# mpeg5/xevd

Hardware: AMD Instinct MI355X
Metric: frames/sec (bit-exact YUV) + achieved HBM GB/s (higher is better)
Workload: dtype s16; 1 GPU; cfg4_main_8k_10b_ra; width=7680, height=4320, bit_depth=10, batches_resident=4, residual_pass_ahead=True, parallelism=1 stream on 1 GPU

## Files before the change

xevd_amd/csrc/itdq_body.h:

```cpp
#pragma once
#include "xgpu_internal.h"

typedef short v2s __attribute__((ext_vector_type(2)));

static __constant__ uint32_t k_tmp[2730];
__host__ __device__ constexpr int tmp_base(int log2n) { return log2n == 1 ? 0 : log2n == 2 ? 2 : log2n == 3 ? 10 : log2n == 4 ? 42 : log2n == 5 ? 170 : 682; }

static __constant__ uint32_t k_atsp[2][680];
__host__ __device__ constexpr int atsp_base(int log2n) { return log2n == 2 ? 0 : log2n == 3 ? 8 : log2n == 4 ? 40 : 168; }

static void upload_transform_tables_tu(const int *tm, const int16_t *ats, hipStream_t s)
{
    static uint32_t apk[2][680];
    for (int t = 0; t < 2; t++) {
        int src = 0;
        for (int l = 2; l <= 5; l++) {
            const int N = 1 << l, dst = atsp_base(l);
            for (int k2 = 0; k2 < N / 2; k2++)
                for (int n = 0; n < N; n++)
                    apk[t][dst + k2 * N + n] = (uint32_t)(uint16_t)ats[t * 1360 + src + (2 * k2) * N + n] |
                                               ((uint32_t)(uint16_t)ats[t * 1360 + src + (2 * k2 + 1) * N + n] << 16);
            src += N * N;
        }
    }
    (void)hipMemcpyToSymbolAsync(HIP_SYMBOL(k_atsp), apk, sizeof(apk), 0, hipMemcpyHostToDevice, s);
    static uint32_t packed[2730];
    int src = 0;
    for (int l = 1; l <= 6; l++) {
        const int N = 1 << l, dst = tmp_base(l);
        for (int k2 = 0; k2 < N / 2; k2++)
            for (int n = 0; n < N; n++)
                packed[dst + k2 * N + n] = (uint32_t)(uint16_t)(int16_t)tm[src + (2 * k2) * N + n] |
                                           ((uint32_t)(uint16_t)(int16_t)tm[src + (2 * k2 + 1) * N + n] << 16);
        src += N * N;
    }
    (void)hipMemcpyToSymbolAsync(HIP_SYMBOL(k_tmp), packed, sizeof(packed), 0, hipMemcpyHostToDevice, s);
    (void)hipStreamSynchronize(s);
}

__device__ __forceinline__ int clip16(int v) { return min(max(v, -32768), 32767); }
__device__ __forceinline__ int dot2(uint32_t a, uint32_t b, int c)
{
    return __builtin_amdgcn_sdot2(__builtin_bit_cast(v2s, a), __builtin_bit_cast(v2s, b), c, false);
}

__host__ __device__ constexpr int itdq_group(int lw, int lh)
{
    const int W = 1 << lw, H = 1 << lh;
    const int l1 = W * (H > 16 ? H / 16 : 1), l2 = H * (W > 16 ? W / 16 : 1);
    return 256 / (l1 > l2 ? l1 : l2);
}

#define ITDQ_PLANES_DWORDS 4608
#define ITDQ_LDS_DWORDS (ITDQ_PLANES_DWORDS + 2048)
#define ITDQ_MAX_G 128

__device__ __forceinline__ uint32_t wave_or(uint32_t v)
{
#pragma unroll
    for (int m = 32; m >= 1; m >>= 1) v |= (uint32_t)__shfl_xor((int)v, m, 64);
    return v;
}

template <int LW, int LH, bool IQT>
__device__ __forceinline__ void itdq_item(const ItdqArgs &a, const TbWave wv, uint32_t *lds, uint32_t *s_rm, uint32_t *s_cm)
{
    constexpr int W = 1 << LW, H = 1 << LH;
    constexpr int N1 = H > 16 ? 16 : H, C1 = H / N1;
    constexpr int N2 = W > 16 ? 16 : W, C2 = W / N2;
    constexpr int G = itdq_group(LW, LH);
    constexpr int RS = W / 2 + 1;
    constexpr int PLANE = G * H * RS;
    constexpr bool UNI1 = (G * W) % 64 == 0, UNI2 = (G * H) % 64 == 0;
    static_assert(2 * PLANE <= ITDQ_PLANES_DWORDS && G * W * H <= 4096 && G <= ITDQ_MAX_G, "LDS budget");
    constexpr int PLANES_DWORDS = IQT ? ITDQ_PLANES_DWORDS / 2 : ITDQ_PLANES_DWORDS;
    constexpr bool RMASK = H >= 16, CMASK = W >= 16;
    const int t = threadIdx.x;
    if (RMASK || CMASK) {
        if (t < G) { s_rm[t] = 0; s_cm[t] = 0; }
        __syncthreads();
    }
    const uint32_t *tmh = (wv.tr_v == TR_DCT2 || LH < 2 || LH > 5) ? k_tmp + tmp_base(LH) : k_atsp[wv.tr_v - 1] + atsp_base(LH);
    const uint32_t *tmw = (wv.tr_h == TR_DCT2 || LW < 2 || LW > 5) ? k_tmp + tmp_base(LW) : k_atsp[wv.tr_h - 1] + atsp_base(LW);
    const bool s16_mid = IQT || wv.tr_v != TR_DCT2 || wv.tr_h != TR_DCT2;
    int16_t *ldsh = (int16_t *)lds;
    int16_t *ldsl = (int16_t *)(lds + PLANE);
    uint32_t *ldsc = lds + PLANES_DWORDS;

    {
        constexpr int S = W * H, UN = S >= 8 ? 8 : 4;
        constexpr int odd = (LW + LH) & 1;
        const int shift = 20 - 14 - (15 - a.bd - ((LW + LH) >> 1)) + (odd ? 8 : 0);
        const long long offset = shift == 0 ? 0 : 1ll << (shift - 1);
        for (int u = t; u < G * S / UN; u += 256) {
            const int p = (u * UN) / S, o = (u * UN) % S;
            if (p >= wv.count) break;
            const TbRec tb = a.tbs[wv.first + p];
            const int qp = tb.qp, sidx = qp % 6;
            const int sbase = sidx == 0 ? 40 : sidx == 1 ? 45 : sidx == 2 ? 51 : sidx == 3 ? 57 : sidx == 4 ? 64 : (IQT ? 72 : 71);
            const long long mul = (long long)(sbase << (qp / 6)) * (odd ? 181 : 1);
            const int16_t *src = a.coef + tb.off + ((o >> LW) << tb.log2s) + (o & (W - 1));
            uint32_t raw[UN / 2];
            if constexpr (UN == 8) { const uint4 v = *(const uint4 *)src; raw[0] = v.x; raw[1] = v.y; raw[2] = v.z; raw[3] = v.w; }
            else { const uint2 v = *(const uint2 *)src; raw[0] = v.x; raw[1] = v.y; }
#pragma unroll
            for (int i = 0; i < UN / 2; i++) {
                if (raw[i] == 0) continue;
                const int c0 = (int16_t)(raw[i] & 0xFFFF), c1 = (int16_t)(raw[i] >> 16);
                const long long l0 = ((long long)c0 * mul + offset) >> shift, l1 = ((long long)c1 * mul + offset) >> shift;
                const int v0 = (int)min(max(l0, -32768ll), 32767ll), v1 = (int)min(max(l1, -32768ll), 32767ll);
                raw[i] = (uint32_t)(uint16_t)v0 | ((uint32_t)(uint16_t)v1 << 16);
                if (RMASK) atomicOr(&s_rm[p], 1u << ((o + 2 * i) >> (LW + 1)));
                if (CMASK) atomicOr(&s_cm[p], 1u << (((o + 2 * i) & (W - 1)) >> 1));
            }
#pragma unroll
            for (int i = 0; i < UN / 2; i++) ldsc[(p * S + o) / 2 + i] = raw[i];
        }
    }
    __syncthreads();

    uint32_t rows1 = 0;
    if (RMASK) {
        const int p1 = (t % (G * W)) >> LW;
        rows1 = (uint32_t)__builtin_amdgcn_readfirstlane((int)wave_or((t < G * W * C1 && p1 < wv.count) ? s_rm[p1] : 0u));
    }
    if (t < G * W * C1) {
        const int idx = t % (G * W);
        int chunk = t / (G * W);
        if (UNI1) chunk = __builtin_amdgcn_readfirstlane(chunk);
        const int p = idx >> LW, j = idx & (W - 1);
        const bool valid = p < wv.count;
        const int16_t *src = (const int16_t *)ldsc + p * (W * H) + j;

        int acc[N1];
#pragma unroll
        for (int n = 0; n < N1; n++) acc[n] = 0;
        if (RMASK) {
            for (uint32_t m = rows1; m; m &= m - 1) {
                const int k2 = __builtin_ctz(m);
                const uint32_t vp = valid ? ((uint32_t)(uint16_t)src[(2 * k2) * W] | ((uint32_t)(uint16_t)src[(2 * k2 + 1) * W] << 16)) : 0u;
                const uint32_t *row = tmh + k2 * H + chunk * N1;
#pragma unroll
                for (int n = 0; n < N1; n++) acc[n] = dot2(row[n], vp, acc[n]);
            }
        } else {
            for (int k2 = 0; k2 < H / 2; k2++) {
                const uint32_t vp = valid ? ((uint32_t)(uint16_t)src[(2 * k2) * W] | ((uint32_t)(uint16_t)src[(2 * k2 + 1) * W] << 16)) : 0u;
                if (__ballot(vp != 0) == 0) continue;
                const uint32_t *row = tmh + k2 * H + chunk * N1;
#pragma unroll
                for (int n = 0; n < N1; n++) acc[n] = dot2(row[n], vp, acc[n]);
            }
        }
        const int base = (p * H + chunk * N1) * (2 * RS) + j;
        if (CMASK && !(valid && ((s_cm[p] >> (j >> 1)) & 1))) {
        } else if (s16_mid) {
#pragma unroll
            for (int n = 0; n < N1; n++) ldsh[base + n * (2 * RS)] = (int16_t)clip16((acc[n] + 64) >> 7);
        } else {
#pragma unroll
            for (int n = 0; n < N1; n++) {
                ldsh[base + n * (2 * RS)] = (int16_t)(acc[n] >> 15);
                ldsl[base + n * (2 * RS)] = (int16_t)(acc[n] & 0x7FFF);
            }
        }
    }
    __syncthreads();

    uint32_t cols2 = 0;
    if (CMASK) {
        const int p2 = (t % (G * H)) >> LH;
        cols2 = (uint32_t)__builtin_amdgcn_readfirstlane((int)wave_or((t < G * H * C2 && p2 < wv.count) ? s_cm[p2] : 0u));
    }
    if (t < G * H * C2) {
        const int idx = t % (G * H);
        int chunk = t / (G * H);
        if (UNI2) chunk = __builtin_amdgcn_readfirstlane(chunk);
        const int p = idx >> LH, r = idx & (H - 1);
        if (p >= wv.count) return;
        const uint32_t own = CMASK ? s_cm[p] : 0xFFFFFFFFu;
        const TbRec tb = a.tbs[wv.first + p];
        const int shift2 = s16_mid ? 12 - (a.bd - 8) : 7 + 12 - (a.bd - 8);
        const uint32_t *inh = lds + (p * H + r) * RS;
        const uint32_t *inl = inh + PLANE;
        int res[N2];
        if (s16_mid) {
            int s[N2];
#pragma unroll
            for (int n = 0; n < N2; n++) s[n] = 1 << (shift2 - 1);
            if (CMASK) {
                for (uint32_t m = cols2; m; m &= m - 1) {
                    const int k2 = __builtin_ctz(m);
                    const uint32_t vp = ((own >> k2) & 1) ? inh[k2] : 0u;
                    const uint32_t *row = tmw + k2 * W + chunk * N2;
#pragma unroll
                    for (int n = 0; n < N2; n++) s[n] = dot2(row[n], vp, s[n]);
                }
            } else {
                for (int k2 = 0; k2 < W / 2; k2++) {
                    const uint32_t vp = inh[k2];
                    if (__ballot(vp != 0) == 0) continue;
                    const uint32_t *row = tmw + k2 * W + chunk * N2;
#pragma unroll
                    for (int n = 0; n < N2; n++) s[n] = dot2(row[n], vp, s[n]);
                }
            }
#pragma unroll
            for (int n = 0; n < N2; n++) res[n] = clip16(s[n] >> shift2);
        } else {
            int sh[N2], sl[N2];
#pragma unroll
            for (int n = 0; n < N2; n++) { sh[n] = 0; sl[n] = 0; }
            if (CMASK) {
                for (uint32_t m = cols2; m; m &= m - 1) {
                    const int k2 = __builtin_ctz(m);
                    const bool mine = (own >> k2) & 1;
                    const uint32_t vh = mine ? inh[k2] : 0u, vl = mine ? inl[k2] : 0u;
                    const uint32_t *row = tmw + k2 * W + chunk * N2;
#pragma unroll
                    for (int n = 0; n < N2; n++) { sh[n] = dot2(row[n], vh, sh[n]); sl[n] = dot2(row[n], vl, sl[n]); }
                }
            } else {
                for (int k2 = 0; k2 < W / 2; k2++) {
                    const uint32_t vh = inh[k2], vl = inl[k2];
                    if (__ballot((vh | vl) != 0) == 0) continue;
                    const uint32_t *row = tmw + k2 * W + chunk * N2;
#pragma unroll
                    for (int n = 0; n < N2; n++) { sh[n] = dot2(row[n], vh, sh[n]); sl[n] = dot2(row[n], vl, sl[n]); }
                }
            }
            const long long add = 1ll << (shift2 - 1);
#pragma unroll
            for (int n = 0; n < N2; n++) {
                const long long s = (long long)sh[n] * 32768 + sl[n] + add;
                res[n] = (int)min(max(s >> shift2, -32768ll), 32767ll);
            }
        }
        int16_t *out = a.resid + tb.off + (r << tb.log2s) + chunk * N2;
        if constexpr (N2 >= 8) {
#pragma unroll
            for (int n = 0; n < N2; n += 8) {
                uint4 v;
                v.x = (uint32_t)(uint16_t)res[n + 0] | ((uint32_t)(uint16_t)res[n + 1] << 16);
                v.y = (uint32_t)(uint16_t)res[n + 2] | ((uint32_t)(uint16_t)res[n + 3] << 16);
                v.z = (uint32_t)(uint16_t)res[n + 4] | ((uint32_t)(uint16_t)res[n + 5] << 16);
                v.w = (uint32_t)(uint16_t)res[n + 6] | ((uint32_t)(uint16_t)res[n + 7] << 16);
                *(uint4 *)(out + n) = v;
            }
        } else if constexpr (N2 == 4) {
            uint2 v;
            v.x = (uint32_t)(uint16_t)res[0] | ((uint32_t)(uint16_t)res[1] << 16);
            v.y = (uint32_t)(uint16_t)res[2] | ((uint32_t)(uint16_t)res[3] << 16);
            *(uint2 *)out = v;
        } else {
            *(uint32_t *)out = (uint32_t)(uint16_t)res[0] | ((uint32_t)(uint16_t)res[1] << 16);
        }
    }
}

template <bool IQT>
__device__ __forceinline__ void itdq_dispatch(const ItdqArgs &a, int wi, uint32_t *lds, uint32_t *s_rm, uint32_t *s_cm)
{
    const TbWave wv = a.waves[wi];
#define CASE(lw, lh) case (lw) * 8 + (lh): itdq_item<lw, lh, IQT>(a, wv, lds, s_rm, s_cm); break;
#define ROW(lw) CASE(lw, 1) CASE(lw, 2) CASE(lw, 3) CASE(lw, 4) CASE(lw, 5) CASE(lw, 6)
    switch (wv.log2w * 8 + wv.log2h) {
        ROW(1) ROW(2) ROW(3) ROW(4) ROW(5) ROW(6)
        default: break;
    }
#undef ROW
#undef CASE
}
```

xevd_amd/csrc/k_intra.hip:

```cpp
#include "xgpu_internal.h"
#include "itdq_body.h"

#include <type_traits>
#include "intra_pred.h"

#define INTRA_WAVES 8


__constant__ uint8_t k_htdf_tbl[5][16] = {
    { 0, 0, 2,  6, 10, 14, 19, 23, 28, 32,  36,  41,  45,  49,  53,  57 },
    { 0, 0, 5, 12, 20, 29, 38, 47, 56, 65,  73,  82,  90,  98, 107, 115 },
    { 0, 0, 1,  4,  9, 16, 24, 32, 41, 50,  59,  68,  77,  86,  94, 103 },
    { 0, 0, 3,  9, 19, 32, 47, 64, 81, 99, 117, 135, 154, 179, 205, 230 },
    { 0, 0, 0,  2,  6, 11, 18, 27, 38, 51,  64,  96, 128, 160, 192, 224 },
};
#define HTDF_EXT (66 * 66)

template <bool HTDF> struct IntraLds { static constexpr int WAVE = (HTDF && HTDF_EXT > 3 * NB_LEN) ? HTDF_EXT : 3 * NB_LEN; };

#ifdef INTRA_PROFILE
__device__ uint32_t g_intra_prof[8 * 64];
#define ISTAMP(k) do { if (DEP && t == 0 && item >= INTRA_PROFILE && item < INTRA_PROFILE + 64) g_intra_prof[8 * (item - INTRA_PROFILE) + (k)] = (uint32_t)clock64(); } while (0)
#else
#define ISTAMP(k)
// ... 533 lines not shown
        if (n > 32) {
            for (int e = 2 * t + 32; e < n; e += 32)
                *(uint32_t *)&nb[c][SB_C0 + 1 + e] = ((avail_up >> (e >> ush)) & 1) ? *(const uint32_t *)(org - s + e) : midp;
            for (int e = t + 32; e < n; e += 16)
                nb[c][SB_C0 - 1 - e] = ((avail_le >> (e >> ush)) & 1) ? org[e * s - 1] : (int16_t)mid;
        }
    }
    wave_lds_sync();
#pragma unroll
    for (int c = 0; c < 3; c++) {
        const int mode = c ? mode_c : mode_l;
        const int w = c ? cw >> 1 : cw, h = c ? chh >> 1 : chh;
        if (mode == 0) {
            int acc = 0;
            for (int e = t; e < w + h; e += 16) acc += e < h ? nb[c][SB_C0 - 1 - e] : nb[c][SB_C0 + 1 + e - h];
            acc = row_sum16(acc);
            if (t == 0) nb[c][NB_DC] = (int16_t)((acc + w) >> ((c ? lw - 1 : lw) + 1));
        } else if (mode == 4) {
            for (int e = t; e < w + h; e += 16) nb[c][SB_UR + e] = (int16_t)((nb[c][SB_C0 + 1 + e] + nb[c][SB_C0 - 1 - e]) >> 1);
        }
    }
    wave_lds_sync();
    if (!has) return;
    const int x = cu_x + lx, y = cu_y + ly;
    int pl[4][4], pc[2][2][2];
    int vl[7], vc[2][3];
    nb_fetch<7, SB_C0, SB_UR>(nb[0], mode_l, lx, ly, vl);
    nb_fetch<3, SB_C0, SB_UR>(nb[1], mode_c, lx >> 1, ly >> 1, vc[0]);
    nb_fetch<3, SB_C0, SB_UR>(nb[2], mode_c, lx >> 1, ly >> 1, vc[1]);
#pragma unroll
    for (int md = 0; md < 5; md++) {
        if (md == mode_l)
#pragma unroll
            for (int r = 0; r < 4; r++)
#pragma unroll
                for (int q = 0; q < 4; q++) pl[r][q] = vl[nb_sel(md, r, q, 3)];
        if (md == mode_c)
#pragma unroll
            for (int c = 0; c < 2; c++)
#pragma unroll
                for (int r = 0; r < 2; r++)
#pragma unroll
                    for (int q = 0; q < 2; q++) pc[c][r][q] = vc[c][nb_sel(md, r, q, 1)];
    }
    int16_t *dy = a.cur_y + y * a.s_l + x;
    const int coff = (y >> 1) * a.s_c + (x >> 1);
    if (!(nflags & 32u))
#pragma unroll
        for (int r = 0; r < 4; r++) {
            const uint32_t o0 = recon2i(pack2i(pl[r][0], pl[r][1]), (cbf & 1) ? rl[r].x : 0u, maxv), o1 = recon2i(pack2i(pl[r][2], pl[r][3]), (cbf & 1) ? rl[r].y : 0u, maxv);
            *(uint2 *)(dy + r * a.s_l) = make_uint2(o0, o1);
        }
    if (!(nflags & 64u))
#pragma unroll
        for (int c = 1; c < 3; c++) {
            int16_t *d = (c == 1 ? a.cur_u : a.cur_v) + coff;
#pragma unroll
            for (int r = 0; r < 2; r++)
                *(uint32_t *)(d + r * a.s_c) = recon2i(pack2i(pc[c - 1][r][0], pc[c - 1][r][1]), ((cbf >> c) & 1) ? rc[c - 1][r] : 0u, maxv);
        }
}

__global__ __launch_bounds__(64 * INTRA_WAVES) void k_intra_l1(const IntraArgs a, uint32_t big)
{
    constexpr int BIG_LDS = INTRA_WAVES * IntraLds<false>::WAVE, SMALL_LDS = SMALL_GROUPS * 3 * SB_LEN;
    __shared__ __attribute__((aligned(16))) int16_t s_nb[BIG_LDS > SMALL_LDS ? BIG_LDS : SMALL_LDS];
    if (blockIdx.x < big) {
        IntraArgs b = a;
        b.count = a.count - a.n_small;
        intra_body<false, 0, false, false, INTRA_WAVES>(b, blockIdx.x, s_nb, nullptr);
    } else intra_small_body(a, blockIdx.x - big, s_nb);
}

template <bool DEP, int EIPD, bool IBC, bool HTDF>
__global__ __launch_bounds__(64 * INTRA_WAVES) void k_intra(const IntraArgs a)
{
    __shared__ __attribute__((aligned(16))) int16_t s_nb[INTRA_WAVES * IntraLds<HTDF>::WAVE];
    __shared__ uint32_t s_chunk;
    intra_body<DEP, EIPD, IBC, HTDF, INTRA_WAVES>(a, blockIdx.x, s_nb, &s_chunk);
}

#define FUSED_WAVES 4
template <int EIPD, bool IBC, bool IQT>
__global__ __launch_bounds__(64 * FUSED_WAVES) void k_intra_itdq(const IntraArgs a, const ItdqArgs r, uint32_t n_intra_wg, uint64_t rate)
{
    constexpr int ITDQ_DW = (IQT ? ITDQ_LDS_DWORDS - ITDQ_PLANES_DWORDS / 2 : ITDQ_LDS_DWORDS) + 2 * ITDQ_MAX_G, INTRA_DW = (FUSED_WAVES * IntraLds<false>::WAVE + 1) / 2 + 4;
    __shared__ __attribute__((aligned(16))) uint32_t raw[ITDQ_DW > INTRA_DW ? ITDQ_DW : INTRA_DW];
    const uint32_t before = min(n_intra_wg, (uint32_t)(((uint64_t)blockIdx.x * rate) >> 32)), after = min(n_intra_wg, (uint32_t)(((uint64_t)(blockIdx.x + 1) * rate) >> 32));
    if (after > before) {
        intra_body<true, EIPD, IBC, false, FUSED_WAVES>(a, blockIdx.x, (int16_t *)raw, raw + INTRA_DW - 1);
    } else {
        const int wi = (int)(blockIdx.x - before);
        if (wi >= r.n_waves) return;
        uint32_t *s_rm = raw + ITDQ_DW - 2 * ITDQ_MAX_G;
        itdq_dispatch<IQT>(r, wi, raw, s_rm, s_rm + ITDQ_MAX_G);
    }
}

void upload_transform_tables_intra(const int *tm, const int16_t *ats, hipStream_t s) { upload_transform_tables_tu(tm, ats, s); }

int intra_chunk(bool with_itdq) { return with_itdq ? FUSED_WAVES : INTRA_WAVES; }

void launch_intra(xgpu_ctx *c, const IntraArgs &a, bool dep, bool ibc, bool htdf, const ItdqArgs *next, bool right)
{
    right = right && c->sp.tool_eipd;
    if (next) {
        const uint32_t n_wg = (uint32_t)((a.count + FUSED_WAVES - 1) / FUSED_WAVES);
        const dim3 g(n_wg + (uint32_t)next->n_waves), b(64 * FUSED_WAVES);
        const uint32_t span = std::max(n_wg, g.x / 2);
        const uint64_t rate = (((uint64_t)n_wg << 32) + span - 1) / span;
#define LAUNCHF(E, I) do { if (next->iqt) hipLaunchKernelGGL((k_intra_itdq<E, I, true>), g, b, 0, c->stream, a, *next, n_wg, rate); else hipLaunchKernelGGL((k_intra_itdq<E, I, false>), g, b, 0, c->stream, a, *next, n_wg, rate); } while (0)
        if (right) LAUNCHF(2, true);
        else if (c->sp.tool_eipd) { if (ibc) LAUNCHF(1, true); else LAUNCHF(1, false); }
        else                 { if (ibc) LAUNCHF(0, true); else LAUNCHF(0, false); }
#undef LAUNCHF
        return;
    }
    const int per = INTRA_WAVES;
    if (!dep && !right && !htdf && !ibc && !c->sp.tool_eipd && a.n_small >= c->intra_small_min) {
        const uint32_t big = (uint32_t)((a.count - a.n_small + per - 1) / per), small_blocks = (uint32_t)((a.n_small + SMALL_GROUPS - 1) / SMALL_GROUPS);
        hipLaunchKernelGGL(k_intra_l1, dim3(big + small_blocks), dim3(64 * INTRA_WAVES), 0, c->stream, a, big);
        return;
    }
    const int blocks = (a.count + per - 1) / per;
    const dim3 g(blocks), b(64 * INTRA_WAVES);
#define LAUNCH(D, E, I, H) hipLaunchKernelGGL((k_intra<D, E, I, H>), g, b, 0, c->stream, a)
    if (right) { if (dep) LAUNCH(true, 2, true, true); else LAUNCH(false, 2, true, true); }
    else if (htdf) {
        if (c->sp.tool_eipd) { if (dep) LAUNCH(true, 1, true, true); else LAUNCH(false, 1, true, true); }
        else                 { if (dep) LAUNCH(true, 0, true, true); else LAUNCH(false, 0, true, true); }
    } else if (ibc) {
        if (c->sp.tool_eipd) { if (dep) LAUNCH(true, 1, true, false); else LAUNCH(false, 1, true, false); }
        else                 { if (dep) LAUNCH(true, 0, true, false); else LAUNCH(false, 0, true, false); }
    } else {
        if (c->sp.tool_eipd) { if (dep) LAUNCH(true, 1, false, false); else LAUNCH(false, 1, false, false); }
        else                 { if (dep) LAUNCH(true, 0, false, false); else LAUNCH(false, 0, false, false); }
    }
#undef LAUNCH
#ifdef INTRA_PROFILE
    static int shots = 0;
    if (dep && ++shots == 5) {
        hipStreamSynchronize(c->stream);
        uint32_t h[8 * 64];
        hipMemcpyFromSymbol(h, HIP_SYMBOL(g_intra_prof), sizeof(h));
        for (int i = 0; i < 64; i++)
            fprintf(stderr, "  pos %d start %10u  wait %6u stage %5u (EIPD luma: issue %5u, return %5u | HTDF: to the block loads %5u from stamp 3, block in LDS %5u) plan %5u predict %5u ack %5u\n", INTRA_PROFILE + i, h[8 * i], h[8 * i + 1] - h[8 * i],
                    h[8 * i + 2] - h[8 * i + 1], h[8 * i + 6] - h[8 * i + 1], h[8 * i + 7] - h[8 * i + 6], h[8 * i + 6] - h[8 * i + 3], h[8 * i + 7] - h[8 * i + 6], h[8 * i + 3] - h[8 * i + 2], h[8 * i + 4] - h[8 * i + 3], h[8 * i + 5] - h[8 * i + 4]);
    }
#endif
}
```

xevd_amd/csrc/k_itdq.hip:

```cpp
#include "itdq_body.h"

template <bool IQT>
__global__ __launch_bounds__(256) void k_itdq(const ItdqArgs a)
{
    __shared__ uint32_t lds[IQT ? ITDQ_LDS_DWORDS - ITDQ_PLANES_DWORDS / 2 : ITDQ_LDS_DWORDS];
    __shared__ uint32_t s_rm[ITDQ_MAX_G], s_cm[ITDQ_MAX_G];
    const int wi = blockIdx.x;
    if (wi >= a.n_waves) return;
    itdq_dispatch<IQT>(a, wi, lds, s_rm, s_cm);
}

int itdq_group_size(int lw, int lh) { return itdq_group(lw, lh); }

void upload_transform_tables_intra(const int *tm, const int16_t *ats, hipStream_t s);
void upload_transform_tables(const int *tm, const int16_t *ats, hipStream_t s)
{
    upload_transform_tables_tu(tm, ats, s);
    upload_transform_tables_intra(tm, ats, s);
}

void launch_itdq(xgpu_ctx *c, const ItdqArgs &a, hipStream_t s)
{
    if (a.n_waves <= 0) return;
    if (a.iqt) hipLaunchKernelGGL(k_itdq<true>, dim3(a.n_waves), dim3(256), 0, s, a);
    else       hipLaunchKernelGGL(k_itdq<false>, dim3(a.n_waves), dim3(256), 0, s, a);
}
```

xevd_amd/csrc/xgpu_api.hip:

```cpp
#include "xgpu_host.h"
#include <memory>

static const int8_t k_chroma_qp_main[58] = { 0, 1, 2, 3, 4, 5, 6, 7, 8, 9, 10, 11, 12, 13, 14, 15, 16, 17, 18, 19, 20, 21, 22, 23, 24, 25, 26, 27, 28, 29,
    29, 30, 31, 32, 33, 34, 35, 36, 37, 37, 38, 39, 40, 40, 41, 42, 43, 44, 45, 46, 47, 48, 49, 50, 51, 52, 53, 54 };
static const int8_t k_chroma_qp_base[58] = {
     0,  1,  2,  3,  4,  5,  6,  7,  8,  9, 10, 11, 12, 13, 14, 15, 16, 17, 18, 19,
    20, 21, 22, 23, 24, 25, 26, 27, 28, 29, 29, 29, 30, 31, 32, 32, 33, 33, 34, 34,
    35, 35, 36, 36, 36, 37, 37, 37, 38, 38, 39, 39, 40, 40, 40, 41, 41, 41 };


const char *xgpu_version(void) { return "xevd_amd 0.1 (gfx950)"; }
const char *xgpu_last_error(const xgpu_ctx *c) { return c ? c->err : "null ctx"; }

void time_begin(xgpu_ctx *c, int k, hipEvent_t *a, hipEvent_t *b)
{
    if (!c->timing) return;
    auto get = [&]() {
        hipEvent_t e;
        if (!c->ev_pool.empty()) { e = c->ev_pool.back(); c->ev_pool.pop_back(); }
        else (void)hipEventCreate(&e);
        return e;
    };
    *a = get(); *b = get();
    (void)hipEventRecord(*a, c->stream);
// ... 6 lines not shown
    c->ev_pending.push_back({ a, b, k });
}
int xgpu_timing_enable(xgpu_ctx *c, int on) { ARGCHK(c, c != NULL); c->timing = on; return XGPU_OK; }
int xgpu_timing_reset(xgpu_ctx *c)
{
    ARGCHK(c, c != NULL);
    HIPCHK(c, hipStreamSynchronize(c->stream));
    for (auto &e : c->ev_pending) { c->ev_pool.push_back(e.a); c->ev_pool.push_back(e.b); }
    c->ev_pending.clear();
    memset(c->t_ms, 0, sizeof(c->t_ms));
    memset(c->t_n, 0, sizeof(c->t_n));
    return XGPU_OK;
}
int xgpu_timing_get(xgpu_ctx *c, double ms[XGPU_K_COUNT], long long n[XGPU_K_COUNT])
{
    ARGCHK(c, c != NULL);
    HIPCHK(c, hipStreamSynchronize(c->stream));
    for (auto &e : c->ev_pending) {
        float t = 0;
        HIPCHK(c, hipEventElapsedTime(&t, e.a, e.b));
        c->t_ms[e.k] += t; c->t_n[e.k]++;
        c->ev_pool.push_back(e.a); c->ev_pool.push_back(e.b);
    }
    c->ev_pending.clear();
    for (int i = 0; i < XGPU_K_COUNT; i++) { ms[i] = c->t_ms[i]; n[i] = c->t_n[i]; }
    return XGPU_OK;
}

static void init_transform_tables(xgpu_ctx *c)
{
    static int tm[5460];
    int o = 0;
    for (int l = 1; l <= 6; l++) {
        const int N = 1 << l;
        for (int k = 0; k < N; k++)
            for (int n = 0; n < N; n++) {
                const double v = k == 0 ? 64.0 : 64.0 * sqrt(2.0) * cos((2 * n + 1) * k * 3.14159265358979323846 / (2.0 * N));
                tm[o++] = (int)(v >= 0 ? floor(v + 0.5) : -floor(-v + 0.5));
            }
    }
    static int16_t ats[2 * 1360];
    for (int t = 0; t < 2; t++) {
        int q = t * 1360;
        for (int l = 2; l <= 5; l++) {
            const int N = 1 << l;
            const double sc = sqrt((double)N) * 64;
            int16_t m[32 * 32];
            for (int k = 0; k < N; k++)
                for (int n = 0; n < N; n++) {
                    const double v = t == 0 ? sin(3.14159265358979323846 * (k + 0.5) * (n + 1) / (N + 0.5)) * sqrt(2.0 / (N + 0.5))
                                            : cos(3.14159265358979323846 * (k + 0.5) * (n + 0.5) / (N + 0.5)) * sqrt(2.0 / (N + 0.5));
                    m[k * N + n] = (int16_t)(sc * v + (v > 0 ? 0.5 : -0.5));
                }
            if (N == 4) {
                const int a = m[0], b = m[1], cc = m[2], d = m[3];
                const int e7[16] = { a, b, cc, b + a,  cc, cc, 0, -cc,  a + b, -a, -cc, b,  b, -(b + a), cc, -a };
                const int e8[16] = { d + cc, b, cc, d,  b, 0, -b, -b,  cc, -b, -d, d + cc,  d, -b, d + cc, -cc };
                for (int i = 0; i < 16; i++) m[i] = (int16_t)(t == 0 ? e7[i] : e8[i]);
            }
            for (int i = 0; i < N * N; i++) ats[q++] = m[i];
        }
    }
    upload_transform_tables(tm, ats, c->stream);
}

int xgpu_open(const xgpu_seq_params *sp, xgpu_ctx **out)
{
    if (!sp || !out) return XGPU_ERR_INVALID_ARGUMENT;
    *out = NULL;
    if (sp->chroma_format_idc != 1) return XGPU_ERR_UNSUPPORTED;
    if (sp->width <= 0 || sp->height <= 0 || (sp->width & 7) || (sp->height & 7)) return XGPU_ERR_INVALID_ARGUMENT;
    if (sp->bit_depth_luma < 8 || sp->bit_depth_luma > 12 || sp->bit_depth_chroma < 8 || sp->bit_depth_chroma > 12) return XGPU_ERR_UNSUPPORTED;
    if (sp->log2_ctu < 5 || sp->log2_ctu > 7) return XGPU_ERR_INVALID_ARGUMENT;
    int ndev = 0;
    if (hipGetDeviceCount(&ndev) != hipSuccess || ndev <= 0 || sp->device < 0 || sp->device >= ndev) return XGPU_ERR_UNEXPECTED;

    xgpu_ctx *c = new xgpu_ctx();
    c->sp = *sp;
    c->sp.chroma_qp_table[0] = c->sp.chroma_qp_table[1] = NULL;
    c->builder_threads = 1;
    c->err[0] = 0; c->timing = 0; c->have_frame = 0; c->side_pic = -1; c->d_maps = NULL; c->d_dra = NULL; c->d_cm = NULL; c->cm_tab = NULL; c->d_ctb_flag = NULL; c->stream = 0; c->up_stream = 0; c->down_stream = 0; c->side_stream = 0; c->after_inter = 0; c->have_after_inter = 0; c->where = 0; c->addb_pending = 0;
    c->fork_ev = c->join_ev = 0;
    c->intra_small_min = getenv("XEVD_HIP_INTRA_SMALL_MIN") ? std::max(1, atoi(getenv("XEVD_HIP_INTRA_SMALL_MIN"))) : 2048;
    c->addb_scalar = getenv("XEVD_HIP_ADDB_SCALAR") != NULL;
    c->split_addb_alf = getenv("XEVD_HIP_SPLIT_ADDB_ALF") != NULL;
    for (int i = 0; i < 2; i++) { c->d_out[i] = NULL; c->out_caps[i] = 0; c->out_ready[i] = c->out_done[i] = 0; c->out_busy[i] = 0; }
    c->d_md5 = NULL; c->md5_ready = 0;
    c->odev_ev[0] = c->odev_ev[1] = 0;
    c->sc_tab = NULL; c->sc_tab_cap = 0; c->sc_mid = NULL; c->sc_mid_cap = 0;
    for (int i = 0; i < 6; i++) c->sc_key[i] = -1;
    c->out_next = 0;
    memset(c->t_ms, 0, sizeof(c->t_ms)); memset(c->t_n, 0, sizeof(c->t_n));
    const int boff = 6 * (sp->bit_depth_chroma - 8);
    for (int t = 0; t < 2; t++)
        for (int q = -boff; q <= 57; q++)
            c->chroma_qp[t][q + boff] = sp->chroma_qp_table[t] ? sp->chroma_qp_table[t][q + boff] : (int8_t)(q < 0 ? q : (sp->tool_iqt ? k_chroma_qp_main[q] : k_chroma_qp_base[q]));

    auto fail = [&](int code) { xgpu_close(c); return code; };
    if (hipSetDevice(sp->device) != hipSuccess) return fail(XGPU_ERR_UNEXPECTED);
    static const bool blocking = getenv("XEVD_HIP_BLOCKING_SYNC") != NULL && atoi(getenv("XEVD_HIP_BLOCKING_SYNC")) != 0;
    if (blocking) (void)hipSetDeviceFlags(hipDeviceScheduleBlockingSync);
    const unsigned ev_flags = hipEventDisableTiming | (blocking ? hipEventBlockingSync : 0);
    {
        static std::atomic<int> n_ctx(0);
        static const bool no_rot = getenv("XEVD_HIP_NO_QUEUE_ROTATION") != NULL;
        const bool swap = !no_rot && (n_ctx.fetch_add(1) & 1);
        hipStream_t *const order[4] = { swap ? &c->side_stream : &c->stream, &c->up_stream, &c->down_stream, swap ? &c->stream : &c->side_stream };
        for (int i = 0; i < 4; i++)
            if (hipStreamCreateWithFlags(order[i], hipStreamNonBlocking) != hipSuccess) return fail(XGPU_ERR_UNEXPECTED);
    }
    if (hipEventCreateWithFlags(&c->after_inter, hipEventDisableTiming) != hipSuccess) return fail(XGPU_ERR_UNEXPECTED);
    if (hipEventCreateWithFlags(&c->fork_ev, hipEventDisableTiming) != hipSuccess || hipEventCreateWithFlags(&c->join_ev, hipEventDisableTiming) != hipSuccess) return fail(XGPU_ERR_UNEXPECTED);
    for (int i = 0; i < 2; i++)
        if (hipEventCreateWithFlags(&c->out_ready[i], hipEventDisableTiming) != hipSuccess || hipEventCreateWithFlags(&c->out_done[i], ev_flags) != hipSuccess)
            return fail(XGPU_ERR_UNEXPECTED);

    c->w_scu = sp->width >> 2; c->h_scu = sp->height >> 2;
    const int ctu = 1 << sp->log2_ctu;
    c->w_ctu = (sp->width + ctu - 1) / ctu; c->h_ctu = (sp->height + ctu - 1) / ctu;
    c->s_l = align_up(XGPU_MARGIN_L + sp->width + XGPU_PAD_L, 64);
    c->s_c = align_up(XGPU_MARGIN_C + (sp->width >> 1) + XGPU_PAD_C, 64);
    c->rows_l = sp->height + 2 * XGPU_PAD_L;
    c->rows_c = (sp->height >> 1) + 2 * XGPU_PAD_C;
    c->off_u = (size_t)c->s_l * c->rows_l;
    c->off_v = c->off_u + (size_t)c->s_c * c->rows_c;
    c->pic_elems = c->off_v + (size_t)c->s_c * c->rows_c + 64;

    if (hipMalloc((void **)&c->d_maps, sizeof(ScuRec) * (size_t)c->w_scu * c->h_scu) != hipSuccess) return fail(XGPU_ERR_OUT_OF_MEMORY);
    if (hipMemsetAsync(c->d_maps, 0, sizeof(ScuRec) * (size_t)c->w_scu * c->h_scu, c->stream) != hipSuccess) return fail(XGPU_ERR_UNEXPECTED);
    if (hipMalloc((void **)&c->d_ctb_flag, (size_t)c->w_ctu * c->h_ctu + 16) != hipSuccess) return fail(XGPU_ERR_OUT_OF_MEMORY);
    init_transform_tables(c);
    c->pics.resize(1 + std::max(1, std::min(sp->max_pics, 34)));
    for (auto &p : c->pics) { p.base = NULL; p.used = 0; }
    {
        DevPic &p = c->pics[0];
        if (hipMalloc((void **)&p.base, c->pic_elems * sizeof(int16_t)) != hipSuccess) return fail(XGPU_ERR_OUT_OF_MEMORY);
        (void)hipMemsetAsync(p.base, 0, c->pic_elems * sizeof(int16_t), c->stream);
        p.s_l = c->s_l; p.s_c = c->s_c; p.used = 1;
        p.y = p.base + (size_t)XGPU_PAD_L * c->s_l + XGPU_MARGIN_L;
        p.u = p.base + c->off_u + (size_t)XGPU_PAD_C * c->s_c + XGPU_MARGIN_C;
        p.v = p.base + c->off_v + (size_t)XGPU_PAD_C * c->s_c + XGPU_MARGIN_C;
    }
    if (hipStreamSynchronize(c->stream) != hipSuccess) return fail(XGPU_ERR_UNEXPECTED);
    *out = c;
    return XGPU_OK;
}

void xgpu_close(xgpu_ctx *c)
{
    if (!c) return;
    (void)hipSetDevice(c->sp.device);
    if (c->stream) (void)hipStreamSynchronize(c->stream);
    if (c->up_stream) (void)hipStreamSynchronize(c->up_stream);
    if (c->down_stream) (void)hipStreamSynchronize(c->down_stream);
    if (c->side_stream) (void)hipStreamSynchronize(c->side_stream);
    for (auto &p : c->pics) if (p.base) (void)hipFree(p.base);
    if (c->d_maps) (void)hipFree(c->d_maps);
    for (BatchBlock &k : c->pool) { (void)hipFree(k.d_base); (void)hipHostFree(k.h_stage); (void)hipEventDestroy(k.uploaded); (void)hipEventDestroy(k.done); (void)hipEventDestroy(k.itdq_done); }
    for (auto &h : c->pinned) (void)hipHostFree(h.p);
    c->pinned.clear();
    c->pool.clear();
    if (c->d_md5) (void)hipFree(c->d_md5);
    if (c->md5_ready) (void)hipEventDestroy(c->md5_ready);
    for (int i = 0; i < 2; i++) if (c->odev_ev[i]) (void)hipEventDestroy(c->odev_ev[i]);
    for (int i = 0; i < 2; i++) { if (c->d_out[i]) (void)hipFree(c->d_out[i]); if (c->out_ready[i]) (void)hipEventDestroy(c->out_ready[i]); if (c->out_done[i]) (void)hipEventDestroy(c->out_done[i]); }
    if (c->d_dra) (void)hipFree(c->d_dra);
// ... 755 lines not shown
```

xevd_amd/csrc/xgpu_internal.h:

```cpp
#pragma once
#include <hip/hip_runtime.h>
#include <stdint.h>
#include <stdio.h>
#include <string.h>
#include <condition_variable>
#include <functional>
#include <mutex>
#include <thread>
#include <vector>
#include "../../include/xevd_hip.h"

#define XGPU_MARGIN_L 192
#define XGPU_MARGIN_C 128

struct DevPic {
    int16_t *base;
    int16_t *y, *u, *v;
    int      s_l, s_c;
    int      used;
};

struct __attribute__((aligned(16))) CuRec {
    uint16_t x, y;
    uint8_t  log2w, log2h;
// ... 212 lines not shown
    BatchBlock blk;
    int        n_cu, n_ctu, n_tb, n_waves;
    size_t     n_coef;
    CuRec     *d_cus;
    uint32_t  *d_ctu_start;
    uint32_t  *d_owner;
    InterItem *d_inter_items;
    uint32_t  *d_inter_work;
    int        n_inter_work;
    int16_t   *d_coef, *d_resid;
    TbRec     *d_tbs;
    TbWave    *d_waves;
    DmvrItem  *d_dmvr_items;
    int16_t   *d_dmvr_mv;
    int        n_dmvr;
    AffItem   *d_aff_items;
    int16_t   *d_cpmv;
    int        n_aff_eif, n_aff_sub;
    IntraRec  *d_intra;
    uint32_t  *d_intra_deps;
    uint32_t  *d_intra_done;
    int        has_ibc, has_htdf;
    int        order_rl;
    int        has_right;
    TileMask   tile_starts;
    int        tiles_across;
    int        n_intra_l1_small;
    int        n_intra, n_levels, n_intra_deps, n_intra_l1, n_intra_heads;
    uint32_t   intra_epoch, intra_tickets;
    void      *h_stage;
    size_t     stage_bytes;
    int        prepared;
    int        upload_waited;
    int        used;
};

struct ScaleTabs { size_t off_first[4], off_count[4], off_w[4]; int stride[4]; int capy, capc; };
struct xgpu_ctx {
    xgpu_seq_params sp;
    int8_t          chroma_qp[2][96];
    hipStream_t     stream;
    hipStream_t     up_stream, down_stream;
    hipStream_t     side_stream;
    hipEvent_t      after_inter;
    int             have_after_inter;
    std::mutex      pool_mu;
    struct HostRange { uint8_t *p; size_t n; };
    std::vector<HostRange> pinned;
    int             w_scu, h_scu, w_ctu, h_ctu;
    int             s_l, s_c, rows_l, rows_c;
    size_t          pic_elems, off_u, off_v;
    std::vector<DevPic> pics;
    ScuRec         *d_maps;
    uint8_t        *d_ctb_flag;
    std::vector<BatchBlock> pool;
    uint8_t        *d_out[2];
    uint8_t        *d_md5;
    hipEvent_t      md5_ready;
    size_t          out_caps[2];
    hipEvent_t      out_ready[2], out_done[2];
    int             out_busy[2], out_next;
    int32_t        *d_dra;
    float          *d_cm;
    xgpu_colour_tables_t *cm_tab;
    xgpu_colour_transform cm_key;
    int             cm_bd;
    uint8_t        *sc_tab;
    size_t          sc_tab_cap;
    int             sc_key[6];
    ScaleTabs       sc_host;
    uint16_t       *sc_mid;
    size_t          sc_mid_cap;
    hipEvent_t      odev_ev[2];
    xgpu_frame_params fp;
    int             have_frame;
    int             side_pic;
    TileMask        no_dbk;
    hipEvent_t      fork_ev, join_ev;
    int             builder_threads;
    int             pad_done;
    int             where;
    int             order_rl;
    int             intra_small_min;
    int             addb_scalar;
    int             addb_pending, split_addb_alf;
    AddbArgs        addb_args;
    int             timing;
    struct Ev { hipEvent_t a, b; int k; };
    std::vector<Ev> ev_pending;
    std::vector<hipEvent_t> ev_pool;
    double          t_ms[XGPU_K_COUNT];
    long long       t_n[XGPU_K_COUNT];
    char            err[256];
};

class WorkPool {
public:
    ~WorkPool() { { std::lock_guard<std::mutex> g(mu); stop = true; } cv.notify_all(); for (std::thread &t : th) t.join(); }
    template <class F> void run(int n, F &&f)
    {
        if (n <= 1) { f(0); return; }
        while ((int)th.size() < n - 1) { const int idx = (int)th.size(); th.emplace_back([this, idx]() { worker(idx); }); }
        const std::function<void(int)> fn = [&f](int k) { f(k); };
        { std::lock_guard<std::mutex> g(mu); job = &fn; want = n - 1; left = n - 1; gen++; }
        cv.notify_all();
        f(0);
        std::unique_lock<std::mutex> g(mu);
        done_cv.wait(g, [this]() { return left == 0; });
        job = nullptr;
    }
private:
    void worker(int idx)
    {
        uint64_t seen = 0;
        for (;;) {
            const std::function<void(int)> *fn = nullptr;
            {
                std::unique_lock<std::mutex> g(mu);
                cv.wait(g, [&]() { return stop || gen != seen; });
                if (stop) return;
                seen = gen;
                if (idx < want) fn = job;
            }
            if (!fn) continue;
            (*fn)(idx + 1);
            std::lock_guard<std::mutex> g(mu);
            if (--left == 0) done_cv.notify_one();
        }
    }
    std::vector<std::thread> th;
    std::mutex mu;
    std::condition_variable cv, done_cv;
    const std::function<void(int)> *job = nullptr;
    int want = 0, left = 0;
    uint64_t gen = 0;
    bool stop = false;
};

void launch_itdq(xgpu_ctx *c, const ItdqArgs &a, hipStream_t s);
void launch_inter(xgpu_ctx *c, const InterArgs &a);
void launch_test_recon(xgpu_ctx *c, const int16_t *coef, const int16_t *pred, int is_coef, int cuw, int cuh, int16_t *rec, int s_rec, int bd);
void launch_test_dbk(xgpu_ctx *c, int16_t *buf, int16_t *buf_v, int st, int st_v, int stride, int bd, int hor, int chroma);
void launch_intra(xgpu_ctx *c, const IntraArgs &a, bool dep, bool ibc, bool htdf, const ItdqArgs *next, bool right = false);
int  intra_chunk(bool with_itdq);
void launch_affine(xgpu_ctx *c, const AffineArgs &a, hipStream_t s);
void launch_dmvr(xgpu_ctx *c, const DmvrArgs &a, hipStream_t s);
void launch_dbk(xgpu_ctx *c, const DbkArgs &a, int dir, const DevPic &src, const DevPic &dst, bool order_rl = false);
void upload_transform_tables(const int *tm, const int16_t *ats, hipStream_t s);
int  itdq_group_size(int log2w, int log2h);
void launch_addb_fused(xgpu_ctx *c, const AddbArgs &a, const DevPic &src, const DevPic &dst);
void launch_alf(xgpu_ctx *c, const AlfArgs &a, const AddbArgs *deblock, const DevPic &src, const DevPic &dst);
void launch_pad(xgpu_ctx *c, const DevPic &p);
void launch_copy_bw(xgpu_ctx *c, const void *src, void *dst, size_t bytes);
void launch_output(xgpu_ctx *c, const DevPic &pic, const int32_t *d_dra, int out_bd, int crop_l, int crop_r, int crop_t, int crop_b, uint8_t *d_dst, bool raw16 = false,
                   hipStream_t s = nullptr);
struct RgbOutArgs {
    const int16_t *y, *u, *v;
    int      sy, sc;
    int      w, h, cw, ch;
    uint8_t *dst;
    size_t   pitch, plane;
    int      aligned;
    int      bgr;
    int      coef[5], shift;
    float    fcoef[5];
    int      yo, co, maxv;
// ... 56 lines not shown
```

Before: 3269 frames/s.

## Process multiple ITDQ waves per workgroup with prefetched coefficients across items

```diff
diff --git a/xevd_amd/csrc/itdq_body.h b/xevd_amd/csrc/itdq_body.h
--- a/xevd_amd/csrc/itdq_body.h
+++ b/xevd_amd/csrc/itdq_body.h
@@ -54,6 +54,48 @@
 #define ITDQ_PLANES_DWORDS 4608
 #define ITDQ_LDS_DWORDS (ITDQ_PLANES_DWORDS + 2048)
 #define ITDQ_MAX_G 128
+#define ITDQ_META_L2S 128
+#define ITDQ_META_RM  160
+#define ITDQ_META_CM  176
+#define ITDQ_MAX_ITEMS 32
+
+struct ItdqPre { uint32_t raw[2][4], off[2], meta[2]; };
+struct ItdqTbs { uint32_t off[2], meta[2]; };
+
+__device__ __forceinline__ bool itdq_unit(int lw, int lh, int count, int t, int s, int &p, int &o)
+{
+    const int ls = lw + lh, unl = ls >= 3 ? 3 : 2;
+    const int gl = 8 - max(lw + max(lh - 4, 0), lh + max(lw - 4, 0));
+    const int u = t + 256 * s, su = u << unl;
+    p = su >> ls; o = su & ((1 << ls) - 1);
+    return u < (1 << (gl + ls - unl)) && p < count;
+}
+
+__device__ __forceinline__ void itdq_fetch_tbs(const ItdqArgs &a, const TbWave wv, bool live, int t, ItdqTbs &q)
+{
+#pragma unroll
+    for (int s = 0; s < 2; s++) {
+        int p, o;
+        itdq_unit(wv.log2w, wv.log2h, live ? wv.count : 0, t, s, p, o);
+        const TbRec tb = a.tbs[wv.first + (uint32_t)max(min(p, (int)wv.count - 1), 0)];
+        q.off[s] = tb.off; q.meta[s] = (uint32_t)tb.qp | ((uint32_t)tb.log2s << 8);
+    }
+}
+
+__device__ __forceinline__ void itdq_fetch_coef(const ItdqArgs &a, const TbWave wv, bool live, int t, const ItdqTbs &q, ItdqPre &pre)
+{
+    const int lw = wv.log2w;
+    const bool small = lw + wv.log2h == 2;
+#pragma unroll
+    for (int s = 0; s < 2; s++) {
+        int p, o;
+        if (!itdq_unit(lw, wv.log2h, live ? wv.count : 0, t, s, p, o)) o = 0;
+        const int16_t *src = a.coef + q.off[s] + ((o >> lw) << (q.meta[s] >> 8)) + (o & ((1 << lw) - 1));
+        if (small) { const uint2 v = *(const uint2 *)src; pre.raw[s][0] = v.x; pre.raw[s][1] = v.y; pre.raw[s][2] = 0; pre.raw[s][3] = 0; }
+        else { const uint4 v = *(const uint4 *)src; pre.raw[s][0] = v.x; pre.raw[s][1] = v.y; pre.raw[s][2] = v.z; pre.raw[s][3] = v.w; }
+        pre.off[s] = q.off[s]; pre.meta[s] = q.meta[s];
+    }
+}
 
 __device__ __forceinline__ uint32_t wave_or(uint32_t v)
 {
@@ -62,9 +104,11 @@
     return v;
 }
 
-template <int LW, int LH, bool IQT>
-__device__ __forceinline__ void itdq_item(const ItdqArgs &a, const TbWave wv, uint32_t *lds, uint32_t *s_rm, uint32_t *s_cm)
-{
+template <int LW, int LH, bool IQT, int PART>
+__device__ __forceinline__ void itdq_item(const ItdqArgs &a, const TbWave wv, ItdqPre &pre, uint32_t *lds, uint32_t *s_meta)
+{
+    uint32_t *s_off = s_meta, *s_rm = s_meta + ITDQ_META_RM, *s_cm = s_meta + ITDQ_META_CM;
+    uint8_t *s_l2s = (uint8_t *)(s_meta + ITDQ_META_L2S);
     constexpr int W = 1 << LW, H = 1 << LH;
     constexpr int N1 = H > 16 ? 16 : H, C1 = H / N1;
     constexpr int N2 = W > 16 ? 16 : W, C2 = W / N2;
@@ -73,36 +117,44 @@
     constexpr int PLANE = G * H * RS;
     constexpr bool UNI1 = (G * W) % 64 == 0, UNI2 = (G * H) % 64 == 0;
     static_assert(2 * PLANE <= ITDQ_PLANES_DWORDS && G * W * H <= 4096 && G <= ITDQ_MAX_G, "LDS budget");
+    static_assert(!(H >= 16 || W >= 16) || G <= 16, "s_meta: 16 mask words per kind");
     constexpr int PLANES_DWORDS = IQT ? ITDQ_PLANES_DWORDS / 2 : ITDQ_PLANES_DWORDS;
     constexpr bool RMASK = H >= 16, CMASK = W >= 16;
-    const int t = threadIdx.x;
+    int t = threadIdx.x;
+    asm volatile("" : "+v"(t));
+    [[maybe_unused]] const uint32_t *tmh = (wv.tr_v == TR_DCT2 || LH < 2 || LH > 5) ? k_tmp + tmp_base(LH) : k_atsp[wv.tr_v - 1] + atsp_base(LH);
+    [[maybe_unused]] const uint32_t *tmw = (wv.tr_h == TR_DCT2 || LW < 2 || LW > 5) ? k_tmp + tmp_base(LW) : k_atsp[wv.tr_h - 1] + atsp_base(LW);
+    [[maybe_unused]] const bool s16_mid = IQT || wv.tr_v != TR_DCT2 || wv.tr_h != TR_DCT2;
+    [[maybe_unused]] int16_t *ldsh = (int16_t *)lds;
+    [[maybe_unused]] int16_t *ldsl = (int16_t *)(lds + PLANE);
+    [[maybe_unused]] uint32_t *ldsc = lds + PLANES_DWORDS;
+
+    if constexpr (PART == 0) {
     if (RMASK || CMASK) {
         if (t < G) { s_rm[t] = 0; s_cm[t] = 0; }
         __syncthreads();
     }
-    const uint32_t *tmh = (wv.tr_v == TR_DCT2 || LH < 2 || LH > 5) ? k_tmp + tmp_base(LH) : k_atsp[wv.tr_v - 1] + atsp_base(LH);
-    const uint32_t *tmw = (wv.tr_h == TR_DCT2 || LW < 2 || LW > 5) ? k_tmp + tmp_base(LW) : k_atsp[wv.tr_h - 1] + atsp_base(LW);
-    const bool s16_mid = IQT || wv.tr_v != TR_DCT2 || wv.tr_h != TR_DCT2;
-    int16_t *ldsh = (int16_t *)lds;
-    int16_t *ldsl = (int16_t *)(lds + PLANE);
-    uint32_t *ldsc = lds + PLANES_DWORDS;
-
     {
         constexpr int S = W * H, UN = S >= 8 ? 8 : 4;
+        constexpr int NU = G * S / UN, SW = NU > 256 ? 2 : 1;
+        static_assert(NU <= 512, "two load units per lane");
         constexpr int odd = (LW + LH) & 1;
         const int shift = 20 - 14 - (15 - a.bd - ((LW + LH) >> 1)) + (odd ? 8 : 0);
         const long long offset = shift == 0 ? 0 : 1ll << (shift - 1);
-        for (int u = t; u < G * S / UN; u += 256) {
+#pragma unroll
+        for (int s = 0; s < SW; s++) asm volatile("" : "+v"(pre.raw[s][0]), "+v"(pre.raw[s][1]), "+v"(pre.raw[s][2]), "+v"(pre.raw[s][3]), "+v"(pre.meta[s]), "+v"(pre.off[s]));
+#pragma unroll
+        for (int s = 0; s < SW; s++) {
+            const int u = t + 256 * s;
             const int p = (u * UN) / S, o = (u * UN) % S;
-            if (p >= wv.count) break;
-            const TbRec tb = a.tbs[wv.first + p];
-            const int qp = tb.qp, sidx = qp % 6;
+            if (u >= NU || p >= wv.count) continue;
+            const int qp = pre.meta[s] & 0xFF, sidx = qp % 6;
             const int sbase = sidx == 0 ? 40 : sidx == 1 ? 45 : sidx == 2 ? 51 : sidx == 3 ? 57 : sidx == 4 ? 64 : (IQT ? 72 : 71);
             const long long mul = (long long)(sbase << (qp / 6)) * (odd ? 181 : 1);
-            const int16_t *src = a.coef + tb.off + ((o >> LW) << tb.log2s) + (o & (W - 1));
+            if (o == 0) { s_off[p] = pre.off[s]; s_l2s[p] = (uint8_t)(pre.meta[s] >> 8); }
             uint32_t raw[UN / 2];
-            if constexpr (UN == 8) { const uint4 v = *(const uint4 *)src; raw[0] = v.x; raw[1] = v.y; raw[2] = v.z; raw[3] = v.w; }
-            else { const uint2 v = *(const uint2 *)src; raw[0] = v.x; raw[1] = v.y; }
+#pragma unroll
+            for (int i = 0; i < UN / 2; i++) raw[i] = pre.raw[s][i];
 #pragma unroll
             for (int i = 0; i < UN / 2; i++) {
                 if (raw[i] == 0) continue;
@@ -117,7 +169,15 @@
             for (int i = 0; i < UN / 2; i++) ldsc[(p * S + o) / 2 + i] = raw[i];
         }
     }
-    __syncthreads();
+    } else {
+    uint32_t cols2 = 0, own = 0xFFFFFFFFu, off2 = 0, l2s2 = 0;
+    const int p2 = (t % (G * H)) >> LH;
+    const bool live2 = t < G * H * C2 && p2 < wv.count;
+    if (live2) { off2 = s_off[p2]; l2s2 = s_l2s[p2]; }
+    if (CMASK) {
+        if (live2) own = s_cm[p2];
+        cols2 = (uint32_t)__builtin_amdgcn_readfirstlane((int)wave_or(live2 ? own : 0u));
+    }
 
     uint32_t rows1 = 0;
     if (RMASK) {
@@ -167,19 +227,11 @@
     }
     __syncthreads();
 
-    uint32_t cols2 = 0;
-    if (CMASK) {
-        const int p2 = (t % (G * H)) >> LH;
-        cols2 = (uint32_t)__builtin_amdgcn_readfirstlane((int)wave_or((t < G * H * C2 && p2 < wv.count) ? s_cm[p2] : 0u));
-    }
-    if (t < G * H * C2) {
+    if (live2) {
         const int idx = t % (G * H);
         int chunk = t / (G * H);
         if (UNI2) chunk = __builtin_amdgcn_readfirstlane(chunk);
-        const int p = idx >> LH, r = idx & (H - 1);
-        if (p >= wv.count) return;
-        const uint32_t own = CMASK ? s_cm[p] : 0xFFFFFFFFu;
-        const TbRec tb = a.tbs[wv.first + p];
+        const int p = p2, r = idx & (H - 1);
         const int shift2 = s16_mid ? 12 - (a.bd - 8) : 7 + 12 - (a.bd - 8);
         const uint32_t *inh = lds + (p * H + r) * RS;
         const uint32_t *inl = inh + PLANE;
@@ -236,7 +288,7 @@
                 res[n] = (int)min(max(s >> shift2, -32768ll), 32767ll);
             }
         }
-        int16_t *out = a.resid + tb.off + (r << tb.log2s) + chunk * N2;
+        int16_t *out = a.resid + off2 + (r << l2s2) + chunk * N2;
         if constexpr (N2 >= 8) {
 #pragma unroll
             for (int n = 0; n < N2; n += 8) {
@@ -256,13 +308,13 @@
             *(uint32_t *)out = (uint32_t)(uint16_t)res[0] | ((uint32_t)(uint16_t)res[1] << 16);
         }
     }
-}
-
-template <bool IQT>
-__device__ __forceinline__ void itdq_dispatch(const ItdqArgs &a, int wi, uint32_t *lds, uint32_t *s_rm, uint32_t *s_cm)
-{
-    const TbWave wv = a.waves[wi];
-#define CASE(lw, lh) case (lw) * 8 + (lh): itdq_item<lw, lh, IQT>(a, wv, lds, s_rm, s_cm); break;
+    }
+}
+
+template <bool IQT, int PART>
+__device__ __forceinline__ void itdq_dispatch(const ItdqArgs &a, const TbWave wv, ItdqPre &pre, uint32_t *lds, uint32_t *s_meta)
+{
+#define CASE(lw, lh) case (lw) * 8 + (lh): itdq_item<lw, lh, IQT, PART>(a, wv, pre, lds, s_meta); break;
 #define ROW(lw) CASE(lw, 1) CASE(lw, 2) CASE(lw, 3) CASE(lw, 4) CASE(lw, 5) CASE(lw, 6)
     switch (wv.log2w * 8 + wv.log2h) {
         ROW(1) ROW(2) ROW(3) ROW(4) ROW(5) ROW(6)
@@ -271,3 +323,51 @@
 #undef ROW
 #undef CASE
 }
+
+template <bool IQT>
+__device__ __forceinline__ void itdq_run(const ItdqArgs &a, int j, int n, int items, uint32_t *lds, uint32_t *s_meta)
+{
+    const int t = threadIdx.x, lane = t & 63;
+    const bool mine = lane < items && j + lane * n < a.n_waves;
+    const int cnt = __builtin_popcountll(__ballot(mine));
+    uint32_t w0 = 0, w1 = 0;
+    if (mine) { const TbWave w = a.waves[j + lane * n]; w0 = w.first; w1 = (uint32_t)w.count | ((uint32_t)w.log2w << 16) | ((uint32_t)w.log2h << 20) | ((uint32_t)w.tr_v << 24) | ((uint32_t)w.tr_h << 28); }
+    auto item = [&](int i) {
+        TbWave wv;
+        const uint32_t x1 = (uint32_t)__builtin_amdgcn_readlane((int)w1, i);
+        wv.first = (uint32_t)__builtin_amdgcn_readlane((int)w0, i);
+        wv.count = (uint16_t)x1; wv.log2w = (uint8_t)((x1 >> 16) & 15); wv.log2h = (uint8_t)((x1 >> 20) & 15); wv.tr_v = (uint8_t)((x1 >> 24) & 15); wv.tr_h = (uint8_t)(x1 >> 28);
+        wv.pad[0] = wv.pad[1] = 0;
+        return wv;
+    };
+    if (cnt == 0) return;
+    TbWave wv = item(0);
+    ItdqTbs tbs;
+    ItdqPre pre;
+    if constexpr (!IQT) {
+        for (int i = 0; i < cnt; i++) {
+            wv = item(i);
+            itdq_fetch_tbs(a, wv, true, t, tbs);
+            itdq_fetch_coef(a, wv, true, t, tbs, pre);
+            itdq_dispatch<IQT, 0>(a, wv, pre, lds, s_meta);
+            __syncthreads();
+            itdq_dispatch<IQT, 1>(a, wv, pre, lds, s_meta);
+        }
+        return;
+    }
+    itdq_fetch_tbs(a, wv, true, t, tbs);
+    itdq_fetch_coef(a, wv, true, t, tbs, pre);
+    TbWave wv1 = item(min(1, cnt - 1));
+    itdq_fetch_tbs(a, wv1, 1 < cnt, t, tbs);
+    for (int i = 0; i < cnt; i++) {
+        const TbWave wv2 = item(min(i + 2, cnt - 1));
+        itdq_dispatch<IQT, 0>(a, wv, pre, lds, s_meta);
+        __syncthreads();
+        if (i + 1 < cnt) {
+            itdq_fetch_coef(a, wv1, true, t, tbs, pre);
+            itdq_fetch_tbs(a, wv2, i + 2 < cnt, t, tbs);
+        }
+        itdq_dispatch<IQT, 1>(a, wv, pre, lds, s_meta);
+        wv = wv1; wv1 = wv2;
+    }
+}
diff --git a/xevd_amd/csrc/k_intra.hip b/xevd_amd/csrc/k_intra.hip
--- a/xevd_amd/csrc/k_intra.hip
+++ b/xevd_amd/csrc/k_intra.hip
@@ -639,7 +639,7 @@
 
 #define FUSED_WAVES 4
 template <int EIPD, bool IBC, bool IQT>
-__global__ __launch_bounds__(64 * FUSED_WAVES) void k_intra_itdq(const IntraArgs a, const ItdqArgs r, uint32_t n_intra_wg, uint64_t rate)
+__global__ __launch_bounds__(64 * FUSED_WAVES) void k_intra_itdq(const IntraArgs a, const ItdqArgs r, uint32_t n_intra_wg, uint64_t rate, int n_resid, int items)
 {
     constexpr int ITDQ_DW = (IQT ? ITDQ_LDS_DWORDS - ITDQ_PLANES_DWORDS / 2 : ITDQ_LDS_DWORDS) + 2 * ITDQ_MAX_G, INTRA_DW = (FUSED_WAVES * IntraLds<false>::WAVE + 1) / 2 + 4;
     __shared__ __attribute__((aligned(16))) uint32_t raw[ITDQ_DW > INTRA_DW ? ITDQ_DW : INTRA_DW];
@@ -647,10 +647,9 @@
     if (after > before) {
         intra_body<true, EIPD, IBC, false, FUSED_WAVES>(a, blockIdx.x, (int16_t *)raw, raw + INTRA_DW - 1);
     } else {
-        const int wi = (int)(blockIdx.x - before);
-        if (wi >= r.n_waves) return;
-        uint32_t *s_rm = raw + ITDQ_DW - 2 * ITDQ_MAX_G;
-        itdq_dispatch<IQT>(r, wi, raw, s_rm, s_rm + ITDQ_MAX_G);
+        const int j = (int)(blockIdx.x - before);
+        if (j >= n_resid) return;
+        itdq_run<IQT>(r, j, n_resid, items, raw, raw + ITDQ_DW - 2 * ITDQ_MAX_G);
     }
 }
 
@@ -663,10 +662,11 @@
     right = right && c->sp.tool_eipd;
     if (next) {
         const uint32_t n_wg = (uint32_t)((a.count + FUSED_WAVES - 1) / FUSED_WAVES);
-        const dim3 g(n_wg + (uint32_t)next->n_waves), b(64 * FUSED_WAVES);
+        const int items = c->itdq_items, n_resid = (next->n_waves + items - 1) / items;
+        const dim3 g(n_wg + (uint32_t)n_resid), b(64 * FUSED_WAVES);
         const uint32_t span = std::max(n_wg, g.x / 2);
         const uint64_t rate = (((uint64_t)n_wg << 32) + span - 1) / span;
-#define LAUNCHF(E, I) do { if (next->iqt) hipLaunchKernelGGL((k_intra_itdq<E, I, true>), g, b, 0, c->stream, a, *next, n_wg, rate); else hipLaunchKernelGGL((k_intra_itdq<E, I, false>), g, b, 0, c->stream, a, *next, n_wg, rate); } while (0)
+#define LAUNCHF(E, I) do { if (next->iqt) hipLaunchKernelGGL((k_intra_itdq<E, I, true>), g, b, 0, c->stream, a, *next, n_wg, rate, n_resid, items); else hipLaunchKernelGGL((k_intra_itdq<E, I, false>), g, b, 0, c->stream, a, *next, n_wg, rate, n_resid, items); } while (0)
         if (right) LAUNCHF(2, true);
         else if (c->sp.tool_eipd) { if (ibc) LAUNCHF(1, true); else LAUNCHF(1, false); }
         else                 { if (ibc) LAUNCHF(0, true); else LAUNCHF(0, false); }
diff --git a/xevd_amd/csrc/k_itdq.hip b/xevd_amd/csrc/k_itdq.hip
--- a/xevd_amd/csrc/k_itdq.hip
+++ b/xevd_amd/csrc/k_itdq.hip
@@ -1,13 +1,11 @@
 #include "itdq_body.h"
 
 template <bool IQT>
-__global__ __launch_bounds__(256) void k_itdq(const ItdqArgs a)
+__global__ __launch_bounds__(256) void k_itdq(const ItdqArgs a, int items)
 {
     __shared__ uint32_t lds[IQT ? ITDQ_LDS_DWORDS - ITDQ_PLANES_DWORDS / 2 : ITDQ_LDS_DWORDS];
-    __shared__ uint32_t s_rm[ITDQ_MAX_G], s_cm[ITDQ_MAX_G];
-    const int wi = blockIdx.x;
-    if (wi >= a.n_waves) return;
-    itdq_dispatch<IQT>(a, wi, lds, s_rm, s_cm);
+    __shared__ uint32_t s_meta[2 * ITDQ_MAX_G];
+    itdq_run<IQT>(a, (int)blockIdx.x, (int)gridDim.x, items, lds, s_meta);
 }
 
 int itdq_group_size(int lw, int lh) { return itdq_group(lw, lh); }
@@ -22,6 +20,7 @@
 void launch_itdq(xgpu_ctx *c, const ItdqArgs &a, hipStream_t s)
 {
     if (a.n_waves <= 0) return;
-    if (a.iqt) hipLaunchKernelGGL(k_itdq<true>, dim3(a.n_waves), dim3(256), 0, s, a);
-    else       hipLaunchKernelGGL(k_itdq<false>, dim3(a.n_waves), dim3(256), 0, s, a);
+    const int items = c->itdq_items, n = (a.n_waves + items - 1) / items;
+    if (a.iqt) hipLaunchKernelGGL(k_itdq<true>, dim3(n), dim3(256), 0, s, a, items);
+    else       hipLaunchKernelGGL(k_itdq<false>, dim3(n), dim3(256), 0, s, a, items);
 }
diff --git a/xevd_amd/csrc/xgpu_api.hip b/xevd_amd/csrc/xgpu_api.hip
--- a/xevd_amd/csrc/xgpu_api.hip
+++ b/xevd_amd/csrc/xgpu_api.hip
@@ -112,6 +112,7 @@
     c->err[0] = 0; c->timing = 0; c->have_frame = 0; c->side_pic = -1; c->d_maps = NULL; c->d_dra = NULL; c->d_cm = NULL; c->cm_tab = NULL; c->d_ctb_flag = NULL; c->stream = 0; c->up_stream = 0; c->down_stream = 0; c->side_stream = 0; c->after_inter = 0; c->have_after_inter = 0; c->where = 0; c->addb_pending = 0;
     c->fork_ev = c->join_ev = 0;
     c->intra_small_min = getenv("XEVD_HIP_INTRA_SMALL_MIN") ? std::max(1, atoi(getenv("XEVD_HIP_INTRA_SMALL_MIN"))) : 2048;
+    c->itdq_items = getenv("XEVD_HIP_ITDQ_ITEMS") ? std::min(32, std::max(1, atoi(getenv("XEVD_HIP_ITDQ_ITEMS")))) : 1;
     c->addb_scalar = getenv("XEVD_HIP_ADDB_SCALAR") != NULL;
     c->split_addb_alf = getenv("XEVD_HIP_SPLIT_ADDB_ALF") != NULL;
     for (int i = 0; i < 2; i++) { c->d_out[i] = NULL; c->out_caps[i] = 0; c->out_ready[i] = c->out_done[i] = 0; c->out_busy[i] = 0; }
diff --git a/xevd_amd/csrc/xgpu_internal.h b/xevd_amd/csrc/xgpu_internal.h
--- a/xevd_amd/csrc/xgpu_internal.h
+++ b/xevd_amd/csrc/xgpu_internal.h
@@ -318,6 +318,7 @@
     int             where;
     int             order_rl;
     int             intra_small_min;
+    int             itdq_items;
     int             addb_scalar;
     int             addb_pending, split_addb_alf;
     AddbArgs        addb_args;
```

Result: slower. 3234 frames/s (-1.1%).
